# fabiocarrara/neural-ode-features

Hardware: AMD Instinct MI355X
Metric: images/sec (fwd+adjoint) CIFAR-10 ODE-ResNet bs=128 at 1/2/4/8 GPU (higher is better)
Workload: dtype f32

## Files before the change

### neural-ode-features_amd/build.py

```python
import os
import subprocess
import sys
from concurrent.futures import ThreadPoolExecutor

HERE = os.path.dirname(os.path.abspath(__file__))
CSRC = os.path.join(HERE, 'csrc')
ROOT = os.path.dirname(HERE)
LIB = os.path.join(CSRC, 'libnode_hip.so')
LIB_DIAG = os.path.join(CSRC, 'libnode_hip_diag.so')
DIAG_SOURCES = ['kernels_w4_bf16.hip', 'kernels_w4_f16.hip', 'w4_select.hip', 'kernels_w4_diag.hip', 'kernels_tiny_solve.hip']
SOURCES = ['kernels_layout.hip', 'kernels_groupnorm.hip', 'kernels_step_control.hip', 'kernels_generic.hip', 'kernels_theta_finalize.hip',
           'kernels_conv_direct.hip', 'kernels_conv_wino1d.hip', 'kernels_conv_wino2d.hip', 'kernels_conv_small.hip', 'conv_select.hip', 'kernels_wgrad.hip', 'kernels_head.hip', 'kernels_loss.hip', 'kernels_optim.hip', 'kernels_w4_pack.hip', 'kernels_w4_f32.hip', 'kernels_w4_bf16.hip', 'kernels_w4_f16.hip', 'kernels_w4_wgrad.hip', 'w4_select.hip', 'kernels_w4s.hip', 'kernels_stem.hip', 'kernels_tiny.hip', 'kernels_tiny_solve.hip', 'kernels_retrieval.hip', 'kernels_svm.hip', 'kernels_augment.hip', 'kernels_resize.hip', 'kernels_imgconv.hip', 'kernels_pool.hip', 'kernels_ministem.hip', 'kernels_attack.hip', 'kernels_batchnorm.hip', 'kernels_bnhead.hip', 'bnfunc_api.hip', 'bnsolve_api.hip', 'bntrunk_api.hip', 'bnstem_api.hip', 'bnhead_api.hip', 'attack_api.hip', 'stem_api.hip', 'trunk_api.hip', 'downconv_api.hip', 'convstem_api.hip', 'ministem_api.hip', 'retrieval_api.hip', 'svm_api.hip', 'augment_api.hip', 'resize_api.hip', 'imgconv_api.hip', 'pool_api.hip', 'host_common.hip', 'dims.hip', 'plan.hip', 'solver.hip', 'api_solve.hip',
           'api_backprop.hip', 'api_flat.hip', 'api_misc.hip']
HEADERS = [os.path.join(CSRC, 'node_internal.h'), os.path.join(CSRC, 'wino4.h'), os.path.join(CSRC, 'w4_gemm.h'), os.path.join(CSRC, 'theta_finalize.h'), os.path.join(CSRC, 'w4s_pass_body.inc'), os.path.join(CSRC, 'conv_common.h'), os.path.join(CSRC, 'pointwise_common.h'), os.path.join(CSRC, 'stem.h'), os.path.join(CSRC, 'batchnorm.h'), os.path.join(CSRC, 'bnfunc.h'), os.path.join(CSRC, 'attack.h'), os.path.join(CSRC, 'stem_plan.h'), os.path.join(CSRC, 'ministem.h'), os.path.join(CSRC, 'step_control.h'), os.path.join(CSRC, 'host_common.h'), os.path.join(CSRC, 'butcher.h'),
           os.path.join(CSRC, 'plan.h'), os.path.join(CSRC, 'solver.h'), os.path.join(ROOT, 'include', 'node_hip.h')]
HIPCC = os.environ.get('HIPCC', '/opt/rocm/bin/hipcc')
FLAGS = ['--offload-arch=gfx950', '-O3', '-fPIC', '-std=c++17', '-Wall', '-Wno-unused-function',
         '-ffp-contract=fast']


def _stale(target, deps):
    if not os.path.exists(target):
        return True
    t = os.path.getmtime(target)
    return any(os.path.getmtime(d) > t for d in deps)


def _compile(src, diag=False):
    obj = os.path.join(CSRC, src.replace('.hip', '.diag.o' if diag else '.o'))
    path = os.path.join(CSRC, src)
    if _stale(obj, [path] + HEADERS):
        cmd = [HIPCC] + FLAGS + (['-DNODE_DIAG'] if diag else []) + ['-c', path, '-o', obj]
        print(' '.join(cmd), flush=True)
# ... 52 lines not shown
```

### neural-ode-features_amd/csrc/kernels_w4_wgrad.hip

```cpp
#include "w4_gemm.h"
#include <cstring>

namespace node {

struct W4WgOps { float4 a0, a1, a2, a3, z; };
template <int NSUB>
__device__ __forceinline__ void w4_wg_mac(float16_t (&acc)[4], const W4WgOps& o, int sub0) {
#define W4WG_STEP(A, ZC)                                                                    \
  if (NSUB == 4) {                                                                           \
    acc[0] = __builtin_amdgcn_mfma_f32_32x32x2f32(A.x, ZC, acc[0], 0, 0, 0);                  \
    acc[1] = __builtin_amdgcn_mfma_f32_32x32x2f32(A.y, ZC, acc[1], 0, 0, 0);                  \
    acc[2] = __builtin_amdgcn_mfma_f32_32x32x2f32(A.z, ZC, acc[2], 0, 0, 0);                  \
    acc[3] = __builtin_amdgcn_mfma_f32_32x32x2f32(A.w, ZC, acc[3], 0, 0, 0);                  \
  } else {                                                                                   \
    acc[0] = __builtin_amdgcn_mfma_f32_32x32x2f32(sub0 ? A.z : A.x, ZC, acc[0], 0, 0, 0);     \
    acc[1] = __builtin_amdgcn_mfma_f32_32x32x2f32(sub0 ? A.w : A.y, ZC, acc[1], 0, 0, 0);     \
  }
  W4WG_STEP(o.a0, o.z.x) W4WG_STEP(o.a1, o.z.y) W4WG_STEP(o.a2, o.z.z) W4WG_STEP(o.a3, o.z.w)
#undef W4WG_STEP
}
__device__ __forceinline__ void w4_wg_load(W4WgOps& o, const float* pa, const float4* pz, int q, size_t rbs) {
  const float4* a = reinterpret_cast<const float4*>(pa + (size_t)(q >> 2) * rbs + (q & 3) * 64);
  o.a0 = a[0]; o.a1 = a[1]; o.a2 = a[2]; o.a3 = a[3];
  o.z = pz[(size_t)q * 64];
// ... 221 lines not shown
#undef W4WG_FETCH
#undef W4WG_WAIT
#undef W4WG_PUT
#undef W4WG_PUT_HALVES
#undef W4WG_F4
#undef W4WG_STASH
  float* o = dU + ((size_t)comp * C + cit * 128) * C + cot * 128 + l31;
#pragma unroll
  for (int r = 0; r < 2; ++r)
#pragma unroll
    for (int c = 0; c < 2; ++c)
#pragma unroll
      for (int q = 0; q < 16; ++q) {
        const int m = (q & 3) + 8 * (q >> 2) + 4 * h;
        st_wt(o + (size_t)(8 * (m >> 1) + 4 * (m & 1) + 2 * wr + r) * C + 32 * (2 * wc + c), acc[r][c][q]);
      }
}

__device__ __forceinline__ void w4wh_dma(const unsigned char* gsrc, unsigned lds_dst) {
  unsigned keep;
  asm volatile("s_mov_b32 %0, m0\n\ts_mov_b32 m0, %2\n\ts_nop 0\n\tglobal_load_lds_dwordx4 %1, off\n\ts_mov_b32 m0, %0"
               : "=&s"(keep) : "v"(gsrc), "s"(lds_dst) : "memory");
}

constexpr int W4WH_NST = 4, W4WH_D = 3, W4WH_STAGE = 16384;
struct W4WgradHArgs {
  const unsigned* V[2]; const unsigned* Z[2];
  float* dU; const Ctrl* ctrl; int N, C, layers;
  const int* v_exp[2]; const int* z_exp;
};
typedef short w4_s16x4 __attribute__((ext_vector_type(4)));
typedef short w4_s16x8 __attribute__((ext_vector_type(8)));
__global__ __launch_bounds__(256, 2) void k_w4_wgrad64h(W4WgradHArgs a) {
  if (a.ctrl != nullptr && a.ctrl->done) return;
  extern __shared__ __attribute__((aligned(16))) unsigned char wsm[];
  const int tid = threadIdx.x, lane = tid & 63, wave = __builtin_amdgcn_readfirstlane(tid >> 6);
  const int C = a.C, nRB = a.N >> 3, G16 = C >> 4, nCT = C >> 7, T = nCT * nCT;
  const int per_xcd = (36 * a.layers) >> 3;
  const int xcd = blockIdx.x & 7, slot = blockIdx.x >> 3;
  const bool by_xcd = ((36 * a.layers) & 7) == 0;
  const int pair = by_xcd ? xcd * per_xcd + slot / T : (int)blockIdx.x / T, tile = by_xcd ? slot % T : (int)blockIdx.x % T;
  const int layer = pair / 36, comp = pair - layer * 36;
  const int cit = tile / nCT, cot = tile - cit * nCT;
  const size_t cbytes = (size_t)nRB * G16 * 2048;
  const unsigned char* Vb = reinterpret_cast<const unsigned char*>(a.V[layer]) + comp * cbytes;
  const unsigned char* Zb = reinterpret_cast<const unsigned char*>(a.Z[layer]) + comp * cbytes;
  const float inv = ldexpf(1.f, -(*a.v_exp[layer] + *a.z_exp));

  const unsigned char* src[4];
#pragma unroll
  for (int k = 0; k < 4; ++k) {
    const int i = 4 * wave + k, isz = i >> 3, g2l = i & 7;
    const int part = lane >> 5, sg = lane & 31, ss = (sg >> 3) ^ (g2l & 1), hi = (sg >> 2) & 1, t = sg & 3;
    const int g2 = (isz ? cot : cit) * 8 + g2l;
    src[k] = (isz ? Zb : Vb) + ((size_t)g2 * 2 + part) * 1024 + ((ss * 2 + hi) * 4 + t) * 16;
  }
  const size_t rb_bytes = (size_t)G16 * 2048;
  const unsigned lds0 = (unsigned)(size_t)(w4_lds_ptr_t)wsm + (unsigned)(4 * wave) * 1024u;
  auto issue = [&](int q) {
    const size_t off = (size_t)(q >> 1) * rb_bytes + (size_t)(q & 1) * 512;
    const unsigned dst = lds0 + (unsigned)(q % W4WH_NST) * W4WH_STAGE;
#pragma unroll
    for (int k = 0; k < 4; ++k) w4wh_dma(src[k] + off, dst + (unsigned)k * 1024u);
  };
  const int wr = wave >> 1, wc = wave & 1;
  const int kh = lane >> 5, g2a = (lane >> 4) & 1, m = lane & 15, q4 = m >> 2, pq = m & 3;
  const int lane_off = (pq & 1) * 64 + q4 * 16 + (pq >> 1) * 8;
  const int s_lo = (2 * kh) ^ g2a, s_hi = (2 * kh + 1) ^ g2a;
  auto frag = [&](const unsigned char* img, int g2l0, int part) -> w4_f16x8 {
    const unsigned char* pb = img + ((g2l0 + g2a) * 2 + part) * 512 + lane_off;
    const w4_s16x4 lo = __builtin_amdgcn_ds_read_tr16_b64_v4i16((__attribute__((address_space(3))) w4_s16x4*)(pb + s_lo * 128));
    const w4_s16x4 hi = __builtin_amdgcn_ds_read_tr16_b64_v4i16((__attribute__((address_space(3))) w4_s16x4*)(pb + s_hi * 128));
    const w4_s16x8 v = {lo[0], lo[1], lo[2], lo[3], hi[0], hi[1], hi[2], hi[3]};
    return __builtin_bit_cast(w4_f16x8, v);
  };
  float16_t acc[2][2];
#pragma unroll
  for (int r = 0; r < 2; ++r)
#pragma unroll
    for (int c = 0; c < 2; ++c)
#pragma unroll
      for (int q = 0; q < 16; ++q) acc[r][c][q] = 0.f;

  const int nK = 2 * nRB;
#pragma unroll
  for (int q = 0; q < W4WH_D; ++q)
    if (q < nK) issue(q);
  for (int q = 0; q < nK; ++q) {
    const int ahead = min(q + W4WH_D - 1, nK - 1) - q;
    if (ahead >= 2) asm volatile("s_waitcnt vmcnt(8)" ::: "memory");
    else if (ahead == 1) asm volatile("s_waitcnt vmcnt(4)" ::: "memory");
    else asm volatile("s_waitcnt vmcnt(0)" ::: "memory");
    asm volatile("s_waitcnt lgkmcnt(0)" ::: "memory");
    __builtin_amdgcn_s_barrier();
    if (q + W4WH_D < nK) issue(q + W4WH_D);
    const unsigned char* st = wsm + (q % W4WH_NST) * W4WH_STAGE;
    w4_f16x8 A[2][2], B[2][2];
#pragma unroll
    for (int r = 0; r < 2; ++r)
#pragma unroll
      for (int part = 0; part < 2; ++part) {
        A[r][part] = frag(st, 4 * wr + 2 * r, part);
        B[r][part] = frag(st + 8192, 4 * wc + 2 * r, part);
      }
#define W4WH_P(AP, BQ)                                                                       \
  _Pragma("unroll") for (int r = 0; r < 2; ++r) _Pragma("unroll") for (int c = 0; c < 2; ++c)  \
      acc[r][c] = __builtin_amdgcn_mfma_f32_32x32x16_f16(A[r][AP], B[c][BQ], acc[r][c], 0, 0, 0);
    W4WH_P(1, 0) W4WH_P(0, 1) W4WH_P(0, 0)
#undef W4WH_P
  }
  float* o = a.dU + ((size_t)layer * 36 + comp) * C * C + (size_t)(cit * 128 + 64 * wr) * C + cot * 128 + 64 * wc + (lane & 31);
#pragma unroll
  for (int r = 0; r < 2; ++r)
#pragma unroll
    for (int c = 0; c < 2; ++c)
#pragma unroll
      for (int q = 0; q < 16; ++q) {
        const int row = (q & 3) + 8 * (q >> 2) + 4 * kh;
        st_wt(o + (size_t)(32 * r + row) * C + 32 * c, acc[r][c][q] * inv);
      }
}
bool w4_wgrad_f16_fits(int N, int C) {
  const W4Switches& sw = w4_switches();
  return sw.f16 != 0 && w4_select_wgrad(sw, N, C, true, W4Operands::Pairs) == W4Wgrad::F16_64;
}
void launch_w4_wgrad_f16(const unsigned* V1, const unsigned* Z1, const unsigned* V2, const unsigned* Z2, float* dU, const Ctrl* ctrl, int N, int C,
                         const int* v1_exp, const int* v2_exp, const int* z_exp, hipStream_t s) {
  static bool attr[MAX_DEVICES] = {};
  W4WgradHArgs a;
  memset(&a, 0, sizeof(a));
  a.V[0] = V1; a.Z[0] = Z1; a.V[1] = V2; a.Z[1] = Z2; a.dU = dU; a.ctrl = ctrl; a.N = N; a.C = C;
  a.layers = V2 != nullptr ? 2 : 1;
  a.v_exp[0] = v1_exp; a.v_exp[1] = v2_exp; a.z_exp = z_exp;
  const int T = (C >> 7) * (C >> 7);
  allow_full_lds(reinterpret_cast<const void*>(k_w4_wgrad64h), attr);
  hipLaunchKernelGGL(k_w4_wgrad64h, dim3(36 * a.layers * T), dim3(256), (size_t)W4WH_NST * W4WH_STAGE, s, a);
}

void launch_w4_wgrad(const W4WgradArgs& a_in, hipStream_t s) {
  const W4Switches& sw = w4_switches();
  W4WgradArgs a = a_in;
  a.sharev = sw.sharev;
  if (w4_select_wgrad(sw, a.N, a.C, a.V2 != nullptr, W4Operands::Fp32) == W4Wgrad::Bf16_128) {
    const int nT = (a.C >> 7) * (a.C >> 7);
    hipLaunchKernelGGL(k_w4_wgrad128b, dim3(8 * (8 * nT + nT)), dim3(256), 2 * 24 * 64 * 16, s, a);
    return;
  }
  const int grid = (a.V2 != nullptr ? 2 : 1) * (a.C >> 7) * (a.C >> 5) * 8;
  const size_t lds = 4 * 2048 * sizeof(float);
  if (a.N % 16 == 0) hipLaunchKernelGGL(k_w4_wgrad<8>, dim3(grid), dim3(256), lds, s, a);
  else hipLaunchKernelGGL(k_w4_wgrad<4>, dim3(grid), dim3(256), lds, s, a);
}

}
```

### neural-ode-features_amd/csrc/node_internal.h

```cpp
#pragma once
#include <hip/hip_runtime.h>
#include <stdint.h>
#include <stddef.h>
#include <cstdlib>
#include "../../include/node_hip.h"

namespace node {

inline int env_int(const char* name, int dflt) {
  const char* e = getenv(name);
  return e ? atoi(e) : dflt;
}

constexpr int KCH = 32;
constexpr int BN = 64;
constexpr int WG_THREADS = 256;

struct Dims {
  int N, C, H, W, HW, G, cpg;
  float eps;
  int Wp, Hp, SLOTS;
  int MARGIN;
  int BNE;
  int ntile;
// ... 371 lines not shown
  float* wpart2;
};
int wgrad_variant();
int wgrad_kernel_for(const Dims& d, int variant);
void launch_wgrad(const Dims& d, const WgradArgs& a, hipStream_t s);
size_t wgrad_lds_bytes(const Dims& d);

struct ThetaFinalizeArgs {
  const float* dU;
  const float* wpart[2];
  const float* spart[2];
  const float* gpart[3];
  int gpart_rows[3];
  int spart_rows;
  const float* wtime[2];
  float* sred;
  EvalTime et;
  float osign;
  float* theta_out;
  Ctrl* ctrl;
  int kidx;
  int write_scalar;
  float* vjp_t_out;
};
void launch_theta_finalize(const Dims& d, const ThetaFinalizeArgs& a, hipStream_t s);

struct TinyConvArgs {
  const float* act;
  const unsigned short* wq;
  const float* bias; const float* tmap;
  EvalTime et;
  const float* gamma; const float* beta;
  float* out;
  float* part; unsigned* counter;
  const Ctrl* ctrl;
  int relu; float osign;
  int nx_on, nx_self;
  Comb nx; float* nx_y_out; const float* nx_gamma; const float* nx_beta; float* nx_act;
};
struct TinyResidentArgs {
  const float* y0;
  float* y_first;
  float* y_out;
  const float* w[2];
  const float* bias[2];
  const float* gamma[3];
// ... 124 lines not shown
```

### neural-ode-features_amd/csrc/solver.h

```cpp
#pragma once
#include "butcher.h"
#include "plan.h"

#include <atomic>

namespace node {

struct StepGuess { int N, C, H, W, aug, forced; float rtol, atol; double t0, t1; int steps; };
int guess_steps(const StepGuess& k);
void remember_steps(const StepGuess& k);

extern int g_w4_pair_stats[4];
extern std::atomic<int> g_resident_cooldown;

struct StepIO {
  int n_targets = 0;
  int n_forced = 0;
  int log_cap = 0;
  float* y_out = nullptr;
  node_step_record* rec = nullptr;
  float* miss_flag = nullptr;
  int expect_steps = 0;
};

// ... 14 lines not shown
  bool w4 = false;
  void choose_w4(bool adaptive) {
    w4 = d.wino4 == 2 || (d.wino4 == 1 && adaptive && rtol >= W4_MIN_TOL && atol >= W4_MIN_TOL && !tiny_mode());
  }
  bool tiny_mode() const { return d.tiny != 0 && !aug && p.wtiny[0] != nullptr; }
  bool small_mode() const { return d.small && !aug && !w4 && p.wsmall[0] != nullptr && !tiny_mode(); }
  bool resident = false;
  void choose_resident(bool dopri5);
  int launch_resident(const float* y0, float* y_out, const StepIO& io, const double* ts, bool inline_targets, bool forced,
                      long long max_steps, int blind);

  bool w4_b16 = false;
  bool w4_f16 = false;
  bool w4_f16_aug = false;
  float* va0_of(int set) const { return (set && p.W4Va0b != nullptr) ? p.W4Va0b : p.W4Va[0]; }
  bool g_ready = false;
  bool f16_now() const { return w4_f16 && (!aug || g_ready); }
  bool v_ready = false;
  int cur = 0;
  float* act1_of(int i) const { return i ? p.act1b : p.act1; }
  float* xh1_of(int i) const { return i ? p.xh1b : p.xh1; }
  float* r1_of(int i) const { return i ? p.r1b : p.r1; }
  bool w4_wgrad_on() const { return w4 && aug && p.W4dU != nullptr; }
  bool theta_rider = true;
  bool tf_waiting = false;
  ThetaFinalizeArgs tf_wait;

  void to_state(const float* nchw, float* dst) {
    if (w4) launch_w4s_from_nchw(nchw, dst, d.N, d.C, d.w4q, st);
    else launch_nchw_to_nhwc(d, nchw, dst, st);
  }
  void from_state(const float* src, float* nchw) {
    if (w4) launch_w4s_to_nchw(src, nchw, d.N, d.C, d.w4q, st);
    else launch_nhwc_to_nchw(d, src, nchw, st);
  }

  void (*nr_fn)(void*, float*, int32_t, void*) = nullptr;
  void* nr_ctx = nullptr;
  float* nr_buf = nullptr;
  float nr_world = 1.f;
  void take_norm_hook(const node_solve_opts* o);
  void norm_exchange(int mode, int nseg);

  double conv_flops() const { return 2.0 * 9.0 * d.C * d.C * (double)d.N * d.HW; }
  int check_launch(const char* what);

// ... 42 lines not shown
```

### neural-ode-features_amd/csrc/solver.hip

```cpp
#include "solver.h"

#include <cmath>
#include <cstring>
#include <mutex>
#include <utility>
#include <vector>

namespace node {

static thread_local std::vector<StepGuess> g_guess;
int guess_steps(const StepGuess& k) {
  for (const auto& g : g_guess)
    if (g.N == k.N && g.C == k.C && g.H == k.H && g.W == k.W && g.aug == k.aug && g.forced == k.forced && g.rtol == k.rtol &&
        g.atol == k.atol && g.t0 == k.t0 && g.t1 == k.t1)
      return g.steps;
  return 1;
}
void remember_steps(const StepGuess& k) {
  for (auto& g : g_guess)
    if (g.N == k.N && g.C == k.C && g.H == k.H && g.W == k.W && g.aug == k.aug && g.forced == k.forced && g.rtol == k.rtol &&
        g.atol == k.atol && g.t0 == k.t0 && g.t1 == k.t1) { g.steps = k.steps; return; }
  if (g_guess.size() >= 64) g_guess.erase(g_guess.begin());
  g_guess.push_back(k);
}
// ... 163 lines not shown
  } else if (d.wino == 2) {
    const float* ws_[4] = {prm.conv1_w, prm.conv2_w, prm.conv1_w, prm.conv2_w};
    float* dst_[4] = {p.wf[0], p.wf[1], p.wd[0], p.wd[1]};
    const int dg_[4] = {0, 0, 1, 1};
    launch_pack_weights_w2_multi(d, ws_, dst_, dg_, aug ? 4 : 2, st);
  } else {
    pack(d, prm.conv1_w, p.wf[0], 0, st);
    pack(d, prm.conv2_w, p.wf[1], 0, st);
    if (aug) {
      pack(d, prm.conv1_w, p.wd[0], 1, st);
      pack(d, prm.conv2_w, p.wd[1], 1, st);
    }
  }
  if (w4 && aug && d.N * d.w4q != d.N8 && p.W4dU != nullptr) {
    for (int i = 0; i < 2; ++i) {
      launch_fill(p.W4Va[i], 0.f, w4_v_elems(d.N8, d.C), st);
      launch_fill(p.W4Z[i], 0.f, w4_z_elems(d.N8, d.C), st);
    }
    launch_fill(p.W4Va0b, 0.f, w4_v_elems(d.N8, d.C), st);
  }
  v_ready = false;
  cur = 0;
  theta_rider = env_int("NODE_TUNE_THETA_RIDER", 1) != 0;
  tf_waiting = false;
  return check_launch("prepare");
}

void Solver::gn_pass_fwd(const float* gamma, const float* beta, int relu, float osign, float* out, float* xhat_out, float* rstd_out) {
  CombineGnArgs ca;
  memset(&ca, 0, sizeof(ca));
  ca.comb.y = p.RAW; ca.comb.nk = 0; ca.comb.scale_mode = SC_ABS; ca.ctrl = p.ctrl;
  ca.act_out = out; ca.xhat_out = xhat_out; ca.rstd_out = rstd_out;
  ca.gamma = gamma; ca.beta = beta; ca.relu = relu; ca.osign = osign;
  launch_combine_gn(d, ca, st);
}
void Solver::gn_pass_bwd(const float* act, const float* xhat, const float* rstd, const float* gamma, float osign, float* out,
                 float* gpart, float* spart) {
  GnBwdArgs g;
  memset(&g, 0, sizeof(g));
  g.comb.y = p.RAW; g.comb.nk = 0; g.comb.scale_mode = SC_ABS; g.ctrl = p.ctrl; g.csign = 1.f;
  g.xhat = xhat; g.rstd = rstd; g.gamma = gamma; g.dz_out = out; g.gpart = gpart; g.spart = spart;
  g.mask_act = act; g.osign = osign;
  launch_gn_bwd(d, g, st);
}

void Solver::w4_gemm(int which, const float* V) {
// ... 135 lines not shown
    W4sArgs a = w4_args();
    a.h.M = p.W4M; a.h.gamma = prm.norm1_w; a.h.beta = prm.norm1_b; a.h.xhat_s = xh1_of(cur); a.h.rstd = r1_of(cur);
    a.h.osign = et.tsign; a.h.out_s = kA_out; a.h.gpart = p.gpart[0];
    if (next != nullptr) {
      w4_tail_combine(a, next->cy, next->y_out, true, cur ^ 1, 0);
      w4_pass(2, 1, a);
      cur ^= 1;
      v_ready = true;
    } else {
      w4_pass(2, 0, a);
    }
  }
  if (!need_theta) return check_launch("augmented dynamics (F(4x4,3x3))");
  ThetaFinalizeArgs tf;
  memset(&tf, 0, sizeof(tf));
  tf.dU = wg4 ? p.W4dU : nullptr;
  tf.wpart[0] = p.wpart[0]; tf.wpart[1] = p.wpart[1];
  tf.spart[0] = p.spart[0]; tf.spart[1] = p.spart[1];
  tf.gpart[0] = p.gpart[0]; tf.gpart[1] = p.gpart[1]; tf.gpart[2] = p.gpart[2];
  tf.gpart_rows[0] = tf.gpart_rows[1] = tf.gpart_rows[2] = tf.spart_rows = d.N * d.w4q;
  tf.wtime[0] = p.wtime[0]; tf.wtime[1] = p.wtime[1]; tf.sred = p.sred;
  tf.et = et; tf.osign = et.tsign; tf.theta_out = kT_out;
  tf.ctrl = p.ctrl; tf.kidx = kidx; tf.write_scalar = kidx >= 0 ? 1 : 0; tf.vjp_t_out = vjp_t_out;
  if (theta_rider && next != nullptr && w4s_rider_fits(d.cpg, d.w4q)) {
    tf_wait = tf;
    tf_waiting = true;
  } else {
    launch_theta_finalize(d, tf, st);
  }
  return check_launch("augmented dynamics (F(4x4,3x3))");
}

int Solver::eval_fwd(const Comb& cy, float* y_out, const EvalTime& et, float* k_out, bool train, const NextComb* next) {
  if (w4) return eval_w4(cy, y_out, et, k_out, train, nullptr, nullptr, nullptr, nullptr, -1, 0.f, nullptr, false, next);
  const bool tiny = tiny_mode() && !train;
  if (!(tiny && v_ready)) {
    CombineGnArgs ca;
    memset(&ca, 0, sizeof(ca));
    ca.comb = cy; ca.ctrl = p.ctrl; ca.y_out = y_out; ca.act_out = p.act1;
    ca.xhat_out = train ? p.xh1 : nullptr; ca.rstd_out = train ? p.r1 : nullptr;
    ca.gamma = prm.norm1_w; ca.beta = prm.norm1_b; ca.relu = 1; ca.osign = 1.f;
    launch_combine_gn(d, ca, st);
  }
  v_ready = false;

  if (tiny) {
// ... 78 lines not shown
    if (d.wgrad_pair) { w1.act2 = p.act2; w1.dz2 = p.dz2; w1.wpart2 = p.wpart[1]; }
    { ProfScope ps(1, (d.wgrad_pair ? 2.0 : 1.0) * conv_flops(), st); launch_wgrad(d, w1, st); }
  }

  ConvArgs b1 = b2;
  b1.spart = nullptr;
  b1.in = p.dz1; b1.wpacked = p.wd[0];
  b1.gamma = prm.norm1_w; b1.osign = et.tsign; b1.out = kA_out;
  b1.act = p.act1; b1.xhat = p.xh1; b1.rstd = p.r1; b1.gpart = p.gpart[0];
  { ProfScope ps(0, conv_flops(), st); launch_conv(d, b1, st); }
  if (d.csplit) gn_pass_bwd(p.act1, p.xh1, p.r1, prm.norm1_w, et.tsign, kA_out, p.gpart[0], nullptr);

  if (!need_theta) return check_launch("augmented dynamics");
  ThetaFinalizeArgs tf;
  memset(&tf, 0, sizeof(tf));
  tf.wpart[0] = p.wpart[0]; tf.wpart[1] = p.wpart[1];
  tf.spart[0] = p.spart[0]; tf.spart[1] = p.spart[1];
  tf.gpart[0] = p.gpart[0]; tf.gpart[1] = p.gpart[1]; tf.gpart[2] = p.gpart[2];
  tf.gpart_rows[0] = tf.gpart_rows[1] = d.csplit ? d.N : d.mtiles;
  tf.gpart_rows[2] = d.N;
  tf.wtime[0] = p.wtime[0]; tf.wtime[1] = p.wtime[1]; tf.sred = p.sred;
  tf.et = et; tf.osign = et.tsign; tf.theta_out = kT_out;
  tf.ctrl = p.ctrl; tf.kidx = kidx; tf.write_scalar = kidx >= 0 ? 1 : 0; tf.vjp_t_out = vjp_t_out;
  launch_theta_finalize(d, tf, st);
  return check_launch("augmented dynamics");
}

int Solver::eval_sys(int kout, const double* coef, int ncoef, int scale_mode, const EvalTime& et, bool write_new,
                     bool need_theta, const double* next_coef, int next_ncoef, bool next_write_new) {
  Comb cy = make_comb(p.Y, p.KY, coef, ncoef, scale_mode);
  NextComb nc;
  const NextComb* next = nullptr;
  if ((w4 || (tiny_mode() && !aug)) && next_coef != nullptr) {
    nc.cy = make_comb(p.Y, p.KY, next_coef, next_ncoef, scale_mode);
    nc.y_out = next_write_new ? p.Y1 : nullptr;
    next = &nc;
  }
  if (!aug) return eval_fwd(cy, write_new ? p.Y1 : nullptr, et, p.KY[kout], false, next);
  Comb ca = make_comb(p.A, p.KA, coef, ncoef, scale_mode);
  return eval_aug(cy, ca, write_new ? p.Y1 : nullptr, write_new ? p.A1 : nullptr, et,
                  p.KY[kout], p.KA[kout], p.KT[kout], kout, -1.f, nullptr, need_theta, next);
}

int Solver::readback() {
  HIP_TRY(hipMemcpyAsync(hctrl, p.ctrl, sizeof(Ctrl), hipMemcpyDeviceToHost, st));
  HIP_TRY(hipStreamSynchronize(st));
// ... 130 lines not shown
```

### neural-ode-features_amd/csrc/theta_finalize.h

```cpp
#pragma once
#include "pointwise_common.h"
#include "wino4.h"

namespace node {

template <typename T>
__device__ __forceinline__ T tf_sel2(const T (&x)[2], int i) { return i ? x[1] : x[0]; }
template <typename T>
__device__ __forceinline__ T tf_sel3(const T (&x)[3], int i) { return i == 0 ? x[0] : i == 1 ? x[1] : x[2]; }

template <int BT>
__device__ __forceinline__ void theta_finalize_body(const ThetaFinalizeArgs& a, const Dims& d, const int bx_all, const int nblk) {
  static_assert(BT == 256 || BT == 128, "a row group is one wave: four of them in one or two per thread");
  __shared__ float red[256];
  __shared__ int s_last;
  const int tid = threadIdx.x;
  const ThetaLayout L = theta_layout(d.C);
  const int C = d.C;
  const int nsm = (9 * C + 63) / 64;
  const int wb = (nblk - 5 * nsm) / 2;
  if (bx_all >= 5 * nsm) {
    const int layer = (bx_all - 5 * nsm) / wb, bx = (bx_all - 5 * nsm) - layer * wb;
    const size_t CC = (size_t)C * C;
    const size_t n4 = 9 * CC / 4;
// ... 46 lines not shown
        const float4 v0 = wp[(size_t)sp * n4 + i], v1 = wp[(size_t)(sp + 1) * n4 + i];
        const float4 v2 = wp[(size_t)(sp + 2) * n4 + i], v3 = wp[(size_t)(sp + 3) * n4 + i];
        acc.x += (v0.x + v1.x) + (v2.x + v3.x); acc.y += (v0.y + v1.y) + (v2.y + v3.y);
        acc.z += (v0.z + v1.z) + (v2.z + v3.z); acc.w += (v0.w + v1.w) + (v2.w + v3.w);
      }
      for (; sp < d.nsplit; ++sp) {
        const float4 v = wp[(size_t)sp * n4 + i];
        acc.x += v.x; acc.y += v.y; acc.z += v.z; acc.w += v.w;
      }
      out[i] = make_float4(a.osign * acc.x, a.osign * acc.y, a.osign * acc.z, a.osign * acc.w);
    }
    return;
  }
  const int job = bx_all / nsm, bxs = bx_all - job * nsm;
  const bool gn = job < 3;
  const int layer = gn ? job : job - 3;
  const int ncol = gn ? 2 * C : 9 * C;
  if (bxs * 64 >= ncol) return;
  const int rows = gn ? tf_sel3(a.gpart_rows, layer) : (a.spart_rows > 0 ? a.spart_rows : d.N);
  const float* src = gn ? tf_sel3(a.gpart, layer) : tf_sel2(a.spart, layer);
  const int cl = tid & 63, rg = tid >> 6;
  const int col = bxs * 64 + cl;
  float vr[256 / BT];
#pragma unroll
  for (int g = 0; g < 256 / BT; ++g) {
    float v = 0.f;
    if (col < ncol) {
      int r = rg + g * (BT / 64);
      for (; r + 12 < rows; r += 16) {
        const float v0 = src[(size_t)r * ncol + col], v1 = src[(size_t)(r + 4) * ncol + col];
        const float v2 = src[(size_t)(r + 8) * ncol + col], v3 = src[(size_t)(r + 12) * ncol + col];
        v += (v0 + v1) + (v2 + v3);
      }
      for (; r < rows; r += 4) v += src[(size_t)r * ncol + col];
    }
    vr[g] = v;
  }
#pragma unroll
  for (int g = 0; g < 256 / BT; ++g) red[g * BT + tid] = vr[g];
  __syncthreads();
  if (rg != 0) return;
  const bool on = col < ncol;
  const float v = (red[cl] + red[64 + cl]) + (red[128 + cl] + red[192 + cl]);
  if (gn) {
    if (on) {
      const int which = col >= C ? 1 : 0;
      a.theta_out[(which ? tf_sel3(L.b, layer) : tf_sel3(L.g, layer)) + (col - which * C)] = a.osign * v;
    }
    return;
  }
  if (on) {
    a.theta_out[tf_sel2(L.wt, layer) + col] = a.osign * (v * eval_time(a.et));
    if (col >= 4 * C && col < 5 * C) a.theta_out[tf_sel2(L.cb, layer) + (col - 4 * C)] = a.osign * v;
  }
  const int nb = (9 * C + 63) / 64;
  float* dotpart = a.sred + (size_t)2 * 9 * C;
  unsigned* counter = reinterpret_cast<unsigned*>(dotpart + 2 * nb);
  const float part = wave_sum(on ? v * tf_sel2(a.wtime, layer)[col] : 0.f);
#if defined(__HIP_DEVICE_COMPILE__) && !defined(__gfx950__)
// ... 29 lines not shown
```

### neural-ode-features_amd/csrc/w4_gemm.h

```cpp
#pragma once
#include "wino4.h"

namespace node {

typedef float float16_t __attribute__((ext_vector_type(16)));
typedef __attribute__((address_space(3))) void* w4_lds_ptr_t;

#ifndef NODE_WT_STORES
#define NODE_WT_STORES 1
#endif
__device__ __forceinline__ void st_wt(float* p, float v) {
#if NODE_WT_STORES
  __hip_atomic_store(p, v, __ATOMIC_RELAXED, __HIP_MEMORY_SCOPE_AGENT);
#else
  *p = v;
#endif
}

typedef __bf16 w4_bf16x8 __attribute__((ext_vector_type(8)));
typedef __bf16 w4_bf16x2 __attribute__((ext_vector_type(2)));
typedef float w4_f32x2 __attribute__((ext_vector_type(2)));
typedef unsigned w4_u32x4 __attribute__((ext_vector_type(4)));
typedef float w4_f32x4 __attribute__((ext_vector_type(4)));
typedef _Float16 w4_f16x8 __attribute__((ext_vector_type(8)));
// ... 113 lines not shown
      w4b_next<NRB>(ring[i], cu);
#pragma unroll
      for (int r = 0; r < NRB; ++r) cur[r] = nxt[r];
    }
  }
  w4_stamp(st, 3);
}

__device__ __forceinline__ void w4c_mac(float16_t (&acc)[2][2], const w4_u32x4 (&a)[2][3], const w4_u32x4 (&b)[2][3]) {
  w4_bf16x8 A[2][3], B[2][3];
#pragma unroll
  for (int r = 0; r < 2; ++r)
#pragma unroll
    for (int q = 0; q < 3; ++q) { A[r][q] = __builtin_bit_cast(w4_bf16x8, a[r][q]); B[r][q] = __builtin_bit_cast(w4_bf16x8, b[r][q]); }
#define W4C_P(AP, BQ)                                                                           \
  _Pragma("unroll") for (int r = 0; r < 2; ++r) _Pragma("unroll") for (int c = 0; c < 2; ++c)   \
      acc[r][c] = __builtin_amdgcn_mfma_f32_32x32x16_bf16(A[r][AP], B[c][BQ], acc[r][c], 0, 0, 0);
  W4C_P(2, 0) W4C_P(0, 2) W4C_P(1, 1) W4C_P(1, 0) W4C_P(0, 1) W4C_P(0, 0)
#undef W4C_P
}

struct W4Switches {
  int g64, b16, sharev, gemm128, wgrad128, f16, h256;
  int early;
  unsigned long long* stamps;
};
const W4Switches& w4_switches();

enum class W4Operands { Fp32, Pairs };
enum class W4Gemm {
  None,
  Small,
  F32Wide,
  F32_64,
  Bf16_64,
  Bf16_128,
  F16_64,
  F16_128,
  F16_256Tail
};
enum class W4Wgrad { None, F32, Bf16_128, F16_64 };
W4Gemm w4_select_gemm(const W4Switches& sw, int N, int C, W4Operands ops);
W4Wgrad w4_select_wgrad(const W4Switches& sw, int N, int C, bool two_layers, W4Operands ops);

void launch_w4_gemm_small(const float* V, const float* U, float* M, const Ctrl* ctrl, const W4Geom& gm, hipStream_t s);
void launch_w4_gemm_f32_wide(const float* V, const float* U, float* M, const Ctrl* ctrl, const W4Geom& gm, hipStream_t s);
// ... 13 lines not shown
```

### neural-ode-features_amd/csrc/w4_select.hip

```cpp
#include "w4_gemm.h"
#include <cstdio>
#include <cstdlib>

namespace node {

#ifdef NODE_DIAG
void w4_diag_switches(W4Switches& sw);
bool launch_w4_gemm_variant(const W4Switches& sw, const float* V, const unsigned short* Ub, float* M, const Ctrl* ctrl, const W4Geom& gm,
                            hipStream_t s);
#else
static void w4_diag_switches(W4Switches&) {}
static bool launch_w4_gemm_variant(const W4Switches&, const float*, const unsigned short*, float*, const Ctrl*, const W4Geom&, hipStream_t) {
  return false;
}
#endif

static W4Switches w4_read_switches() {
  auto rd = env_int;
  W4Switches sw = {rd("NODE_TUNE_W4_GEMM64", 1), rd("NODE_TUNE_W4_BF16X3", 1), rd("NODE_TUNE_W4_SHAREV", 1), rd("NODE_TUNE_W4_GEMM128", -1),
                   rd("NODE_TUNE_W4_WGRAD128", -1), rd("NODE_TUNE_W4_F16", 1), rd("NODE_TUNE_W4_H256", 1), 0, nullptr};
  w4_diag_switches(sw);
  return sw;
}
static thread_local W4Switches g_w4_sw;
static thread_local bool g_w4_sw_valid = false;
void w4_refresh_tuning() { g_w4_sw = w4_read_switches(); g_w4_sw_valid = true; }
const W4Switches& w4_switches() {
  if (!g_w4_sw_valid) w4_refresh_tuning();
  return g_w4_sw;
}

static bool w4_wants_tiled(int sw, int C) { return sw == 1 || (sw < 0 && C >= 512); }
static bool w4_fits_tiles128(int N, int C) { return N % 32 == 0 && C % 128 == 0 && (((N / 32) * (C >> 7)) & 1) == 0; }
static bool w4_fits_tiles256(int N, int C, int h256) { return N % 64 == 0 && C % 256 == 0 && (h256 == 2 || ((N / 64) * (C >> 8)) % 8 == 0); }
static bool w4_reads_triples(W4Gemm k) { return k == W4Gemm::Bf16_64 || k == W4Gemm::Bf16_128; }

W4Gemm w4_select_gemm(const W4Switches& sw, int N, int C, W4Operands ops) {
  if (ops == W4Operands::Fp32) {
    if (N <= 16) return W4Gemm::Small;
    if (sw.g64 == 0 || N % 16 != 0) return W4Gemm::F32Wide;
    if (sw.b16 == 0) return W4Gemm::F32_64;
    return w4_fits_tiles128(N, C) && w4_wants_tiled(sw.gemm128, C) ? W4Gemm::Bf16_128 : W4Gemm::Bf16_64;
  }
// ... 55 lines not shown
```

Baseline: 30010.

## Interleave wgrad DMA issue with MFMAs and batch prefetch loads in theta finalize

Adds a paced variant of the fp16 Winograd weight-gradient kernel. It spreads the global-to-LDS DMA requests for the next stage between MFMA instructions, using scalar base pointers and unrolled four-stage steps, instead of issuing them all right after the barrier. The variant is chosen when the grid has at least two blocks per CU. Separately, the theta-finalize column reduction now loads 16 rows per group into registers before summing, to expose more memory-level parallelism. Both paths are on by default behind env switches, and diag timing stamps are added. The cost is more code and register pressure.

```diff
diff --git a/neural-ode-features_amd/build.py b/neural-ode-features_amd/build.py
--- a/neural-ode-features_amd/build.py
+++ b/neural-ode-features_amd/build.py
@@ -8,7 +8,7 @@
 ROOT = os.path.dirname(HERE)
 LIB = os.path.join(CSRC, 'libnode_hip.so')
 LIB_DIAG = os.path.join(CSRC, 'libnode_hip_diag.so')
-DIAG_SOURCES = ['kernels_w4_bf16.hip', 'kernels_w4_f16.hip', 'w4_select.hip', 'kernels_w4_diag.hip', 'kernels_tiny_solve.hip']
+DIAG_SOURCES = ['kernels_w4_bf16.hip', 'kernels_w4_f16.hip', 'kernels_w4_wgrad.hip', 'w4_select.hip', 'kernels_w4_diag.hip', 'kernels_tiny_solve.hip']
 SOURCES = ['kernels_layout.hip', 'kernels_groupnorm.hip', 'kernels_step_control.hip', 'kernels_generic.hip', 'kernels_theta_finalize.hip',
            'kernels_conv_direct.hip', 'kernels_conv_wino1d.hip', 'kernels_conv_wino2d.hip', 'kernels_conv_small.hip', 'conv_select.hip', 'kernels_wgrad.hip', 'kernels_head.hip', 'kernels_loss.hip', 'kernels_optim.hip', 'kernels_w4_pack.hip', 'kernels_w4_f32.hip', 'kernels_w4_bf16.hip', 'kernels_w4_f16.hip', 'kernels_w4_wgrad.hip', 'w4_select.hip', 'kernels_w4s.hip', 'kernels_stem.hip', 'kernels_tiny.hip', 'kernels_tiny_solve.hip', 'kernels_retrieval.hip', 'kernels_svm.hip', 'kernels_augment.hip', 'kernels_resize.hip', 'kernels_imgconv.hip', 'kernels_pool.hip', 'kernels_ministem.hip', 'kernels_attack.hip', 'kernels_batchnorm.hip', 'kernels_bnhead.hip', 'bnfunc_api.hip', 'bnsolve_api.hip', 'bntrunk_api.hip', 'bnstem_api.hip', 'bnhead_api.hip', 'attack_api.hip', 'stem_api.hip', 'trunk_api.hip', 'downconv_api.hip', 'convstem_api.hip', 'ministem_api.hip', 'retrieval_api.hip', 'svm_api.hip', 'augment_api.hip', 'resize_api.hip', 'imgconv_api.hip', 'pool_api.hip', 'host_common.hip', 'dims.hip', 'plan.hip', 'solver.hip', 'api_solve.hip',
            'api_backprop.hip', 'api_flat.hip', 'api_misc.hip']
diff --git a/neural-ode-features_amd/csrc/kernels_w4_wgrad.hip b/neural-ode-features_amd/csrc/kernels_w4_wgrad.hip
--- a/neural-ode-features_amd/csrc/kernels_w4_wgrad.hip
+++ b/neural-ode-features_amd/csrc/kernels_w4_wgrad.hip
@@ -1,5 +1,7 @@
 #include "w4_gemm.h"
+#include <cstdlib>
 #include <cstring>
+#include <type_traits>
 
 namespace node {
 
@@ -267,15 +269,33 @@
   asm volatile("s_mov_b32 %0, m0\n\ts_mov_b32 m0, %2\n\ts_nop 0\n\tglobal_load_lds_dwordx4 %1, off\n\ts_mov_b32 m0, %0"
                : "=&s"(keep) : "v"(gsrc), "s"(lds_dst) : "memory");
 }
+__device__ __forceinline__ void w4wh_dma_s(unsigned lane_off, const unsigned char* sbase, unsigned lds_dst) {
+  unsigned keep;
+  asm volatile("s_mov_b32 %0, m0\n\ts_mov_b32 m0, %3\n\ts_nop 0\n\tglobal_load_lds_dwordx4 %1, %2\n\ts_mov_b32 m0, %0"
+               : "=&s"(keep) : "v"(lane_off), "s"(sbase), "s"(lds_dst) : "memory");
+}
 
 constexpr int W4WH_NST = 4, W4WH_D = 3, W4WH_STAGE = 16384;
 struct W4WgradHArgs {
   const unsigned* V[2]; const unsigned* Z[2];
   float* dU; const Ctrl* ctrl; int N, C, layers;
   const int* v_exp[2]; const int* z_exp;
+  unsigned long long* stamps;
 };
+#ifdef NODE_DIAG
+#define W4WH_T(K_)                                                             \
+  if (stp != nullptr) {                                                        \
+    if ((K_) == 3) asm volatile("s_waitcnt lgkmcnt(0)" ::: "memory");          \
+    const unsigned long long t_ = clock64();                                   \
+    ph[K_] += t_ - tl;                                                         \
+    tl = t_;                                                                   \
+  }
+#else
+#define W4WH_T(K_)
+#endif
 typedef short w4_s16x4 __attribute__((ext_vector_type(4)));
 typedef short w4_s16x8 __attribute__((ext_vector_type(8)));
+template <bool PACED>
 __global__ __launch_bounds__(256, 2) void k_w4_wgrad64h(W4WgradHArgs a) {
   if (a.ctrl != nullptr && a.ctrl->done) return;
   extern __shared__ __attribute__((aligned(16))) unsigned char wsm[];
@@ -291,23 +311,25 @@
   const unsigned char* Vb = reinterpret_cast<const unsigned char*>(a.V[layer]) + comp * cbytes;
   const unsigned char* Zb = reinterpret_cast<const unsigned char*>(a.Z[layer]) + comp * cbytes;
   const float inv = ldexpf(1.f, -(*a.v_exp[layer] + *a.z_exp));
-
+#ifdef NODE_DIAG
+  unsigned long long* stp = a.stamps != nullptr ? a.stamps + ((size_t)blockIdx.x * 4 + wave) * 16 : nullptr;
+  unsigned long long ph[5] = {0, 0, 0, 0, 0}, tl = 0, t_begin = 0;
+  if (stp != nullptr && lane == 0) stp[6] = wall_clock64();
+#endif
+
+  const unsigned char* opb = wave >= 2 ? Zb : Vb;
+  unsigned loff[4];
   const unsigned char* src[4];
 #pragma unroll
   for (int k = 0; k < 4; ++k) {
     const int i = 4 * wave + k, isz = i >> 3, g2l = i & 7;
     const int part = lane >> 5, sg = lane & 31, ss = (sg >> 3) ^ (g2l & 1), hi = (sg >> 2) & 1, t = sg & 3;
     const int g2 = (isz ? cot : cit) * 8 + g2l;
-    src[k] = (isz ? Zb : Vb) + ((size_t)g2 * 2 + part) * 1024 + ((ss * 2 + hi) * 4 + t) * 16;
+    if constexpr (PACED) loff[k] = (unsigned)((g2 * 2 + part) * 1024 + ((ss * 2 + hi) * 4 + t) * 16);
+    else src[k] = (isz ? Zb : Vb) + ((size_t)g2 * 2 + part) * 1024 + ((ss * 2 + hi) * 4 + t) * 16;
   }
   const size_t rb_bytes = (size_t)G16 * 2048;
   const unsigned lds0 = (unsigned)(size_t)(w4_lds_ptr_t)wsm + (unsigned)(4 * wave) * 1024u;
-  auto issue = [&](int q) {
-    const size_t off = (size_t)(q >> 1) * rb_bytes + (size_t)(q & 1) * 512;
-    const unsigned dst = lds0 + (unsigned)(q % W4WH_NST) * W4WH_STAGE;
-#pragma unroll
-    for (int k = 0; k < 4; ++k) w4wh_dma(src[k] + off, dst + (unsigned)k * 1024u);
-  };
   const int wr = wave >> 1, wc = wave & 1;
   const int kh = lane >> 5, g2a = (lane >> 4) & 1, m = lane & 15, q4 = m >> 2, pq = m & 3;
   const int lane_off = (pq & 1) * 64 + q4 * 16 + (pq >> 1) * 8;
@@ -328,32 +350,136 @@
       for (int q = 0; q < 16; ++q) acc[r][c][q] = 0.f;
 
   const int nK = 2 * nRB;
-#pragma unroll
-  for (int q = 0; q < W4WH_D; ++q)
-    if (q < nK) issue(q);
-  for (int q = 0; q < nK; ++q) {
-    const int ahead = min(q + W4WH_D - 1, nK - 1) - q;
-    if (ahead >= 2) asm volatile("s_waitcnt vmcnt(8)" ::: "memory");
-    else if (ahead == 1) asm volatile("s_waitcnt vmcnt(4)" ::: "memory");
-    else asm volatile("s_waitcnt vmcnt(0)" ::: "memory");
-    asm volatile("s_waitcnt lgkmcnt(0)" ::: "memory");
-    __builtin_amdgcn_s_barrier();
-    if (q + W4WH_D < nK) issue(q + W4WH_D);
-    const unsigned char* st = wsm + (q % W4WH_NST) * W4WH_STAGE;
-    w4_f16x8 A[2][2], B[2][2];
-#pragma unroll
-    for (int r = 0; r < 2; ++r)
-#pragma unroll
-      for (int part = 0; part < 2; ++part) {
-        A[r][part] = frag(st, 4 * wr + 2 * r, part);
-        B[r][part] = frag(st + 8192, 4 * wc + 2 * r, part);
-      }
+#ifdef NODE_DIAG
+  if (stp != nullptr) { tl = clock64(); t_begin = tl; }
+#endif
+  if constexpr (PACED) {
+    const unsigned char* nxt = opb;
+    int nxt_odd = 0;
+    auto request = [&](int pk, unsigned dst) { w4wh_dma_s(loff[pk], nxt, dst + (unsigned)pk * 1024u); };
+    auto advance = [&]() {
+      nxt += nxt_odd ? rb_bytes - 512 : (size_t)512;
+      nxt_odd ^= 1;
+    };
+#pragma unroll
+    for (int q = 0; q < W4WH_D; ++q)
+      if (q < nK) {
+#pragma unroll
+        for (int k = 0; k < 4; ++k) request(k, lds0 + (unsigned)q * W4WH_STAGE);
+        advance();
+      }
+    auto step = [&](int stage, auto fill, auto vm) {
+      constexpr bool FILL = decltype(fill)::value;
+      constexpr int VM = decltype(vm)::value;
+      asm volatile("s_waitcnt vmcnt(%0)" ::"n"(VM) : "memory");
+      asm volatile("s_waitcnt lgkmcnt(0)" ::: "memory");
+      W4WH_T(0)
+      __builtin_amdgcn_s_barrier();
+      W4WH_T(1)
+      const unsigned char* st = wsm + stage * W4WH_STAGE;
+      const unsigned dst = lds0 + (unsigned)((stage + W4WH_D) % W4WH_NST) * W4WH_STAGE;
+      w4_f16x8 A[2][2], B[2][2];
+#pragma unroll
+      for (int r = 0; r < 2; ++r)
+#pragma unroll
+        for (int part = 0; part < 2; ++part) {
+          A[r][part] = frag(st, 4 * wr + 2 * r, part);
+          B[r][part] = frag(st + 8192, 4 * wc + 2 * r, part);
+        }
+      W4WH_T(3)
+      if constexpr (FILL) __builtin_amdgcn_sched_barrier(0);
+#pragma unroll
+      for (int n = 0; n < 12; ++n) {
+        const int p = n >> 2, r = (n >> 1) & 1, c = n & 1;
+        const int ap = p == 0 ? 1 : 0, bq = p == 1 ? 1 : 0;
+        acc[r][c] = __builtin_amdgcn_mfma_f32_32x32x16_f16(A[r][ap], B[c][bq], acc[r][c], 0, 0, 0);
+        if constexpr (FILL) {
+          if (n % 3 == 1) {
+            __builtin_amdgcn_sched_barrier(0);
+            request(n / 3, dst);
+            __builtin_amdgcn_sched_barrier(0);
+          }
+        }
+      }
+      if constexpr (FILL) advance();
+      W4WH_T(4)
+    };
+    using Fill = std::true_type;
+    using Tail = std::false_type;
+    using Vm8 = std::integral_constant<int, 8>;
+    using Vm4 = std::integral_constant<int, 4>;
+    using Vm0 = std::integral_constant<int, 0>;
+    int q = 0;
+    for (; q + W4WH_D + 3 < nK; q += 4) {
+      step(0, Fill(), Vm8());
+      step(1, Fill(), Vm8());
+      step(2, Fill(), Vm8());
+      step(3, Fill(), Vm8());
+    }
+    if (q + W4WH_D < nK) {
+      step(0, Fill(), Vm8());
+      if (++q + W4WH_D < nK) {
+        step(1, Fill(), Vm8());
+        if (++q + W4WH_D < nK) {
+          step(2, Fill(), Vm8());
+          ++q;
+        }
+      }
+    }
+    int stage = q & (W4WH_NST - 1);
+    const int rem = nK - q;
+    if (rem >= 3) { step(stage, Tail(), Vm8()); stage = (stage + 1) & (W4WH_NST - 1); }
+    if (rem >= 2) { step(stage, Tail(), Vm4()); stage = (stage + 1) & (W4WH_NST - 1); }
+    step(stage, Tail(), Vm0());
+  } else {
+    auto issue = [&](int q) {
+      const size_t off = (size_t)(q >> 1) * rb_bytes + (size_t)(q & 1) * 512;
+      const unsigned dst = lds0 + (unsigned)(q % W4WH_NST) * W4WH_STAGE;
+#pragma unroll
+      for (int k = 0; k < 4; ++k) w4wh_dma(src[k] + off, dst + (unsigned)k * 1024u);
+    };
+#pragma unroll
+    for (int q = 0; q < W4WH_D; ++q)
+      if (q < nK) issue(q);
+    for (int q = 0; q < nK; ++q) {
+      const int ahead = min(q + W4WH_D - 1, nK - 1) - q;
+      if (ahead >= 2) asm volatile("s_waitcnt vmcnt(8)" ::: "memory");
+      else if (ahead == 1) asm volatile("s_waitcnt vmcnt(4)" ::: "memory");
+      else asm volatile("s_waitcnt vmcnt(0)" ::: "memory");
+      asm volatile("s_waitcnt lgkmcnt(0)" ::: "memory");
+      W4WH_T(0)
+      __builtin_amdgcn_s_barrier();
+      W4WH_T(1)
+      if (q + W4WH_D < nK) issue(q + W4WH_D);
+      W4WH_T(2)
+      const unsigned char* st = wsm + (q % W4WH_NST) * W4WH_STAGE;
+      w4_f16x8 A[2][2], B[2][2];
+#pragma unroll
+      for (int r = 0; r < 2; ++r)
+#pragma unroll
+        for (int part = 0; part < 2; ++part) {
+          A[r][part] = frag(st, 4 * wr + 2 * r, part);
+          B[r][part] = frag(st + 8192, 4 * wc + 2 * r, part);
+        }
+      W4WH_T(3)
 #define W4WH_P(AP, BQ)                                                                       \
   _Pragma("unroll") for (int r = 0; r < 2; ++r) _Pragma("unroll") for (int c = 0; c < 2; ++c)  \
       acc[r][c] = __builtin_amdgcn_mfma_f32_32x32x16_f16(A[r][AP], B[c][BQ], acc[r][c], 0, 0, 0);
-    W4WH_P(1, 0) W4WH_P(0, 1) W4WH_P(0, 0)
+      W4WH_P(1, 0) W4WH_P(0, 1) W4WH_P(0, 0)
 #undef W4WH_P
-  }
+      W4WH_T(4)
+    }
+  }
+#ifdef NODE_DIAG
+  if (stp != nullptr && lane == 0) {
+    unsigned hw, xcc;
+    asm volatile("s_getreg_b32 %0, hwreg(HW_REG_HW_ID)" : "=s"(hw));
+    asm volatile("s_getreg_b32 %0, hwreg(HW_REG_XCC_ID)" : "=s"(xcc));
+#pragma unroll
+    for (int k = 0; k < 5; ++k) stp[k] = ph[k];
+    stp[7] = wall_clock64(); stp[8] = hw; stp[9] = xcc; stp[10] = clock64() - t_begin;
+  }
+#endif
   float* o = a.dU + ((size_t)layer * 36 + comp) * C * C + (size_t)(cit * 128 + 64 * wr) * C + cot * 128 + 64 * wc + (lane & 31);
 #pragma unroll
   for (int r = 0; r < 2; ++r)
@@ -365,21 +491,40 @@
         st_wt(o + (size_t)(32 * r + row) * C + 32 * c, acc[r][c][q] * inv);
       }
 }
+#undef W4WH_T
 bool w4_wgrad_f16_fits(int N, int C) {
   const W4Switches& sw = w4_switches();
   return sw.f16 != 0 && w4_select_wgrad(sw, N, C, true, W4Operands::Pairs) == W4Wgrad::F16_64;
 }
 void launch_w4_wgrad_f16(const unsigned* V1, const unsigned* Z1, const unsigned* V2, const unsigned* Z2, float* dU, const Ctrl* ctrl, int N, int C,
                          const int* v1_exp, const int* v2_exp, const int* z_exp, hipStream_t s) {
-  static bool attr[MAX_DEVICES] = {};
+  static bool attr[2][MAX_DEVICES] = {};
+  const W4Switches& sw = w4_switches();
   W4WgradHArgs a;
   memset(&a, 0, sizeof(a));
   a.V[0] = V1; a.Z[0] = Z1; a.V[1] = V2; a.Z[1] = Z2; a.dU = dU; a.ctrl = ctrl; a.N = N; a.C = C;
   a.layers = V2 != nullptr ? 2 : 1;
   a.v_exp[0] = v1_exp; a.v_exp[1] = v2_exp; a.z_exp = z_exp;
+#ifdef NODE_DIAG
+  const char* e = getenv("NODE_TUNE_W4_WGRAD_STAMPS");
+  a.stamps = e != nullptr ? reinterpret_cast<unsigned long long*>(strtoull(e, nullptr, 0)) : nullptr;
+#endif
   const int T = (C >> 7) * (C >> 7);
-  allow_full_lds(reinterpret_cast<const void*>(k_w4_wgrad64h), attr);
-  hipLaunchKernelGGL(k_w4_wgrad64h, dim3(36 * a.layers * T), dim3(256), (size_t)W4WH_NST * W4WH_STAGE, s, a);
+  static int cus[MAX_DEVICES] = {};
+  int dev = 0, ncu = 256;
+  (void)hipGetDevice(&dev);
+  if (dev >= 0 && dev < MAX_DEVICES) {
+    if (cus[dev] == 0 && hipDeviceGetAttribute(&cus[dev], hipDeviceAttributeMultiprocessorCount, dev) != hipSuccess) { (void)hipGetLastError(); cus[dev] = 256; }
+    ncu = cus[dev];
+  }
+  const bool paced = sw.wgrad_paced > 0 || (sw.wgrad_paced < 0 && 36 * a.layers * T >= 2 * ncu);
+  if (paced) {
+    allow_full_lds(reinterpret_cast<const void*>(k_w4_wgrad64h<true>), attr[1]);
+    hipLaunchKernelGGL(k_w4_wgrad64h<true>, dim3(36 * a.layers * T), dim3(256), (size_t)W4WH_NST * W4WH_STAGE, s, a);
+    return;
+  }
+  allow_full_lds(reinterpret_cast<const void*>(k_w4_wgrad64h<false>), attr[0]);
+  hipLaunchKernelGGL(k_w4_wgrad64h<false>, dim3(36 * a.layers * T), dim3(256), (size_t)W4WH_NST * W4WH_STAGE, s, a);
 }
 
 void launch_w4_wgrad(const W4WgradArgs& a_in, hipStream_t s) {
diff --git a/neural-ode-features_amd/csrc/node_internal.h b/neural-ode-features_amd/csrc/node_internal.h
--- a/neural-ode-features_amd/csrc/node_internal.h
+++ b/neural-ode-features_amd/csrc/node_internal.h
@@ -417,6 +417,7 @@
   int kidx;
   int write_scalar;
   float* vjp_t_out;
+  int prefetch;
 };
 void launch_theta_finalize(const Dims& d, const ThetaFinalizeArgs& a, hipStream_t s);
 
diff --git a/neural-ode-features_amd/csrc/solver.h b/neural-ode-features_amd/csrc/solver.h
--- a/neural-ode-features_amd/csrc/solver.h
+++ b/neural-ode-features_amd/csrc/solver.h
@@ -60,6 +60,7 @@
   float* xh1_of(int i) const { return i ? p.xh1b : p.xh1; }
   float* r1_of(int i) const { return i ? p.r1b : p.r1; }
   bool w4_wgrad_on() const { return w4 && aug && p.W4dU != nullptr; }
+  bool tf_prefetch = true;
   bool theta_rider = true;
   bool tf_waiting = false;
   ThetaFinalizeArgs tf_wait;
diff --git a/neural-ode-features_amd/csrc/solver.hip b/neural-ode-features_amd/csrc/solver.hip
--- a/neural-ode-features_amd/csrc/solver.hip
+++ b/neural-ode-features_amd/csrc/solver.hip
@@ -209,6 +209,7 @@
   v_ready = false;
   cur = 0;
   theta_rider = env_int("NODE_TUNE_THETA_RIDER", 1) != 0;
+  tf_prefetch = env_int("NODE_TUNE_TF_PREFETCH", 1) != 0;
   tf_waiting = false;
   return check_launch("prepare");
 }
@@ -390,6 +391,7 @@
   tf.wtime[0] = p.wtime[0]; tf.wtime[1] = p.wtime[1]; tf.sred = p.sred;
   tf.et = et; tf.osign = et.tsign; tf.theta_out = kT_out;
   tf.ctrl = p.ctrl; tf.kidx = kidx; tf.write_scalar = kidx >= 0 ? 1 : 0; tf.vjp_t_out = vjp_t_out;
+  tf.prefetch = tf_prefetch ? 1 : 0;
   if (theta_rider && next != nullptr && w4s_rider_fits(d.cpg, d.w4q)) {
     tf_wait = tf;
     tf_waiting = true;
@@ -514,6 +516,7 @@
   tf.wtime[0] = p.wtime[0]; tf.wtime[1] = p.wtime[1]; tf.sred = p.sred;
   tf.et = et; tf.osign = et.tsign; tf.theta_out = kT_out;
   tf.ctrl = p.ctrl; tf.kidx = kidx; tf.write_scalar = kidx >= 0 ? 1 : 0; tf.vjp_t_out = vjp_t_out;
+  tf.prefetch = tf_prefetch ? 1 : 0;
   launch_theta_finalize(d, tf, st);
   return check_launch("augmented dynamics");
 }
diff --git a/neural-ode-features_amd/csrc/theta_finalize.h b/neural-ode-features_amd/csrc/theta_finalize.h
--- a/neural-ode-features_amd/csrc/theta_finalize.h
+++ b/neural-ode-features_amd/csrc/theta_finalize.h
@@ -92,19 +92,52 @@
   const int cl = tid & 63, rg = tid >> 6;
   const int col = bxs * 64 + cl;
   float vr[256 / BT];
+  if (a.prefetch) {
+    constexpr int G = 256 / BT;
+    const int wrg = __builtin_amdgcn_readfirstlane(rg);
 #pragma unroll
-  for (int g = 0; g < 256 / BT; ++g) {
-    float v = 0.f;
+    for (int g = 0; g < G; ++g) vr[g] = 0.f;
     if (col < ncol) {
-      int r = rg + g * (BT / 64);
-      for (; r + 12 < rows; r += 16) {
-        const float v0 = src[(size_t)r * ncol + col], v1 = src[(size_t)(r + 4) * ncol + col];
-        const float v2 = src[(size_t)(r + 8) * ncol + col], v3 = src[(size_t)(r + 12) * ncol + col];
-        v += (v0 + v1) + (v2 + v3);
+      const float* colp = src + col;
+      for (int r0 = 0; r0 < rows; r0 += 64) {
+        float x[G][16];
+#pragma unroll
+        for (int g = 0; g < G; ++g)
+#pragma unroll
+          for (int k = 0; k < 16; ++k) {
+            const int r = r0 + wrg + g * (BT / 64) + 4 * k;
+            x[g][k] = colp[(size_t)min(r, rows - 1) * ncol];
+          }
+#pragma unroll
+        for (int g = 0; g < G; ++g)
+#pragma unroll
+          for (int j = 0; j < 4; ++j) {
+            const int r = r0 + wrg + g * (BT / 64) + 16 * j;
+            if (r + 12 < rows) {
+              vr[g] += (x[g][4 * j] + x[g][4 * j + 1]) + (x[g][4 * j + 2] + x[g][4 * j + 3]);
+            } else {
+#pragma unroll
+              for (int i = 0; i < 4; ++i)
+                if (r + 4 * i < rows) vr[g] += x[g][4 * j + i];
+            }
+          }
       }
-      for (; r < rows; r += 4) v += src[(size_t)r * ncol + col];
     }
-    vr[g] = v;
+  } else {
+#pragma unroll
+    for (int g = 0; g < 256 / BT; ++g) {
+      float v = 0.f;
+      if (col < ncol) {
+        int r = rg + g * (BT / 64);
+        for (; r + 12 < rows; r += 16) {
+          const float v0 = src[(size_t)r * ncol + col], v1 = src[(size_t)(r + 4) * ncol + col];
+          const float v2 = src[(size_t)(r + 8) * ncol + col], v3 = src[(size_t)(r + 12) * ncol + col];
+          v += (v0 + v1) + (v2 + v3);
+        }
+        for (; r < rows; r += 4) v += src[(size_t)r * ncol + col];
+      }
+      vr[g] = v;
+    }
   }
 #pragma unroll
   for (int g = 0; g < 256 / BT; ++g) red[g * BT + tid] = vr[g];
diff --git a/neural-ode-features_amd/csrc/w4_gemm.h b/neural-ode-features_amd/csrc/w4_gemm.h
--- a/neural-ode-features_amd/csrc/w4_gemm.h
+++ b/neural-ode-features_amd/csrc/w4_gemm.h
@@ -159,6 +159,7 @@
 
 struct W4Switches {
   int g64, b16, sharev, gemm128, wgrad128, f16, h256;
+  int wgrad_paced;
   int early;
   unsigned long long* stamps;
 };
diff --git a/neural-ode-features_amd/csrc/w4_select.hip b/neural-ode-features_amd/csrc/w4_select.hip
--- a/neural-ode-features_amd/csrc/w4_select.hip
+++ b/neural-ode-features_amd/csrc/w4_select.hip
@@ -18,7 +18,8 @@
 static W4Switches w4_read_switches() {
   auto rd = env_int;
   W4Switches sw = {rd("NODE_TUNE_W4_GEMM64", 1), rd("NODE_TUNE_W4_BF16X3", 1), rd("NODE_TUNE_W4_SHAREV", 1), rd("NODE_TUNE_W4_GEMM128", -1),
-                   rd("NODE_TUNE_W4_WGRAD128", -1), rd("NODE_TUNE_W4_F16", 1), rd("NODE_TUNE_W4_H256", 1), 0, nullptr};
+                   rd("NODE_TUNE_W4_WGRAD128", -1), rd("NODE_TUNE_W4_F16", 1), rd("NODE_TUNE_W4_H256", 1),
+                   rd("NODE_TUNE_W4_WGRAD_PACED", -1), 0, nullptr};
   w4_diag_switches(sw);
   return sw;
 }
```

Measured after the change: 30090 (median of 2 runs). No clear change (+0.2%).
